# spotify/basic-pitch

Hardware: AMD Instinct MI355X
Metric: audio windows/sec (2 s @ 22.05 kHz) end-to-end CQT+CNN (higher is better)
Workload: dtype f32 I/O + accumulate, split-f16 (22-bit hi+lo) MFMA operands, all three products of every layer on f16 MFMA; 1 GPU; batch=256 synthetic uniform[-1,1) 2 s @ 22.05 kHz mono windows per GPU, fp32, HBM-resident in/out (BASELINE.json configs[1])

## Files before the change

### basic_pitch_amd/_native.py

```python
from __future__ import annotations

import ctypes as C
import os
from typing import Optional

from . import build as _build

BP_OK = 0
BP_ERR_INVALID_ARG = -1
BP_ERR_OUT_OF_MEMORY = -5
BP_ERR_UNSUPPORTED = -6
BP_ERR_BAD_AUDIO = -7
BP_MEM_HOST = 0
BP_MEM_DEVICE = 1
BP_FLAG_STAGE_TIMING = 1
BP_FLAG_TIME_DOMINANT = 16
BP_FLAG_F32_MFMA = 2
BP_FLAG_BF16_WEIGHTS = 4
BP_FLAG_EXT_CQT_44K = 8
BP_FLAG_F16_CORRECTIONS = 32
BP_FLAG_FP8_CORRECTIONS = 64
BP_FLAG_BLOCKING_WAIT = 128
BP_PCM_F32, BP_PCM_S16, BP_PCM_S24, BP_PCM_S32, BP_PCM_U8, BP_PCM_F64 = range(6)
BP_PCM_S16_BE, BP_PCM_S24_BE, BP_PCM_S32_BE, BP_PCM_F32_BE, BP_PCM_F64_BE, BP_PCM_S8, BP_PCM_ULAW, BP_PCM_ALAW = range(6, 14)
# ... 36 lines not shown
        ("compute_units", C.c_int),
        ("max_windows", C.c_int64),
        ("workspace_bytes", C.c_int64),
        ("arch", C.c_char * 32),
    ]


class bp_stage_buffers(C.Structure):
    _fields_ = [
        ("audio", C.c_void_p),
        ("pyr", C.c_void_p),
        ("lp", C.c_void_p),
        ("mm", C.c_void_p),
        ("c1", C.c_void_p),
        ("contour", C.c_void_p),
        ("n1", C.c_void_p),
        ("note", C.c_void_p),
        ("o1", C.c_void_p),
        ("onset", C.c_void_p),
        ("zp", C.c_void_p),
    ]


class bp_launch_plan_out(C.Structure):

    _fields_ = [(name, C.c_int32) for name in (
        "pyramid_one_launch", "pyramid_decimate_grid", "pyramid_decimate_grid_cap", "filterbank_fused", "filterbank_grid",
        "conv1_chunks", "conv1_grid", "conv1_prio", "rim_march", "rim_items", "rim_per_side", "rim_items_max", "rim_items_min",
        "rim_ring", "conv2_slots", "conv2_launches", "conv2_windows", "conv2_first_windows", "conv2_first_groups",
        "conv2_first_slabs", "conv2_first_slab_rows", "conv2_first_grid", "conv2_last_windows", "conv2_last_groups",
        "conv2_last_slabs", "conv2_last_slab_rows", "conv2_last_grid", "note_grid", "note_grid_cap", "note_prio", "note_aligned",
        "note_share_spans_pairs", "onset_grid", "onset_grid_cap", "onset_prio", "onset_aligned", "onset_share_spans_pairs",
        "conv2_fused", "fused_cols", "fused_seam_rows", "fused_term_rows", "fused_window_floats", "finish_slabs",
        "finish_slab_rows", "finish_grid")]


class bp_note_params(C.Structure):
    _fields_ = [
        ("onset_threshold", C.c_double),
        ("frame_threshold", C.c_double),
        ("min_freq_hz", C.c_double),
        ("max_freq_hz", C.c_double),
        ("min_note_len", C.c_int32),
        ("infer_onsets", C.c_int32),
        ("melodia_trick", C.c_int32),
        ("include_pitch_bends", C.c_int32),
        ("energy_tol", C.c_int32),
        ("reserved", C.c_int32),
    ]


class bp_flac_stream_layout(C.Structure):
    _fields_ = [
        ("channels", C.c_int32),
        ("sample_rate", C.c_int32),
        ("bits_per_sample", C.c_int32),
        ("min_block", C.c_int32),
        ("max_block", C.c_int32),
        ("n_frames", C.c_int64),
        ("audio_start", C.c_int64),
    ]


class bp_pcm_file_layout(C.Structure):
    _fields_ = [
        ("container", C.c_int32),
        ("format", C.c_int32),
# ... 659 lines not shown
```

### basic_pitch_amd/csrc/bp_api.hip

```cpp
#include <cmath>
#include <cstring>
#include <ctime>

#include "bp_context.h"
#include "cqt_planes.h"
#include "launch_plan.h"
#include "weight_pack.h"

namespace bp {
static void launch_onset(const uint32_t* zp, const float* note, const void* wfrag, const float* wf32, const void* w16,
                         float* onset, int n_windows, int n_cu, bool weights_have_lo, hipStream_t stream) {
#ifdef BP_AB_KERNELS
  static const int kind = [] {
    const char* e = ab_env("BP_ONSET");
    return e && std::strcmp(e, "ring") == 0 ? 2 : (e && std::strcmp(e, "march32") == 0 ? 1 : 0);
  }();
  if (kind == 1) {
    launch_onset_march(zp, note, wfrag, wf32, onset, n_windows, n_cu, weights_have_lo, stream);
    return;
  }
  if (kind == 2) {
    launch_onset_branch(zp, note, wfrag, wf32, onset, n_windows, n_cu, weights_have_lo, stream);
    return;
  }
// ... 83 lines not shown
static void launch_rim(bp_handle h, const uint32_t* zp, float* c1, int n, bool wlo, hipStream_t s) {
  static const bool gemm = [] {
    const char* e = ab_env("BP_RIM");
    return e && std::strcmp(e, "gemm") == 0;
  }();
  if (h->ext || gemm || !h->d_d1_wrimm)
    launch_contour_conv1_rim(zp, h->d_d1_wrim, h->d_d1_bias.as<float>(), c1, n, h->n_cu, wlo, h->ext, s);
  else
    launch_contour_conv1_rim_march(zp, h->d_d1_wrimm, h->d_d1_bias.as<float>(), c1, n, h->n_cu, wlo, s);
}

static bool contour_fused(bp_handle h) {
  static const bool unfused = [] {
    const char* e = ab_env("BP_CONV2");
    return e && (std::strcmp(e, "unfused") == 0 || std::strcmp(e, "valu") == 0);
  }();
  return !h->ext && !unfused && contour_conv1_use_march();
}

static void launch_conv1_interior(bp_handle h, const uint32_t* zp, float* c1, int n, bool wlo, hipStream_t s) {
#ifdef BP_AB_KERNELS
  if (!contour_conv1_use_march()) {
    launch_contour_conv1_folded(zp, h->d_d1_wfold, h->d_d1_bias.as<float>(), c1, n, h->n_cu, wlo, s);
    return;
  }
#endif
  if (contour_fused(h))
    launch_contour_conv1_march(zp, h->d_d1_wmarch, h->d_d1_bias.as<float>(), h->c1, h->d_d2_w.as<float>(), n, h->n_cu, wlo, s);
  else
    launch_contour_conv1_march(zp, h->d_d1_wmarch, h->d_d1_bias.as<float>(), c1, nullptr, n, h->n_cu, wlo, s);
}

static void launch_conv2_of(bp_handle h, float* contour, int n, bool wlo, hipStream_t s) {
  if (contour_fused(h))
    launch_contour_conv2_finish(h->c1s, h->c1, h->d_d2_wproj, h->b_contour2, contour, n, h->n_cu, wlo, s);
  else
    launch_conv2(h->c1s, h->d_d2_w.as<float>(), h->d_d2_wproj, h->b_contour2, contour, n, h->n_cu, wlo, s);
}

static int64_t pyr_level_off(bp_handle h, int k) {
  return h->ext ? ((k == 1) ? 0 : kAudioN + pyr_off(k - 1)) : pyr_off(k);
}

}

namespace bp {

int run_chunk(bp_handle h, const float* audio_dev, int n, float* note_dev, float* onset_dev,
              float* contour_dev) {
  hipStream_t s = h->stream;
  const bool timing = (h->flags & BP_FLAG_STAGE_TIMING) != 0;
  const bool dom = !timing && (h->flags & BP_FLAG_TIME_DOMINANT) && !(h->flags & BP_FLAG_F32_MFMA) &&
                   (h->dom_chunks++ % bp_context::kDomEvery) == 0;
  const bool wlo = !(h->flags & BP_FLAG_BF16_WEIGHTS);
  int e = dom ? -1 : 0;
  const int ring_slot = (int)(h->timed_chunks % bp_context::kTimedRing);
  hipEvent_t* ev = h->ev[ring_slot];
  int* seq = h->seq[ring_slot];
  if (timing) BP_HIP(hipEventRecord(ev[0], s));
#define BP_DOM_BEGIN()                                \
  do {                                                \
    if (dom) {                                        \
      if (e >= 0) seq[e] = -1;                        \
      BP_HIP(hipEventRecord(ev[e + 1], s));           \
      ++e;                                            \
    }                                                 \
// ... 426 lines not shown
  const PlGeo g = make_pl_geo(ext);
  std::memset(out, 0, sizeof *out);
  out->pyramid_one_launch = pyramid_one_launch(n, n_cu, ext);
  out->pyramid_decimate_grid = out->pyramid_one_launch ? 0 : pyramid_decimate_grid((g.len[1] + kPlTileOut - 1) / kPlTileOut, n, n_cu);
  out->pyramid_decimate_grid_cap = pl_resident_waves(n_cu) / kPlDecimateWaves;
  out->filterbank_fused = filterbank_fused(true, n, n_cu);
  out->filterbank_grid = filterbank_grid(out->filterbank_fused != 0, n, n * g.n_levels * kPlTilesPerLevel, n_cu);
  out->conv1_chunks = contour_march_chunks(n, n_cu);
  out->conv1_grid = contour_march_grid(n * out->conv1_chunks * kCmStrips, n_cu);
  out->conv1_prio = march_prio(kCmPrio, out->conv1_grid, n_cu);
  out->rim_march = !ext;
  if (!ext) {
    out->rim_items = n * kRmTiles;
    out->rim_per_side = rim_march_per_side(out->rim_items, n_cu);
    out->rim_items_max = rim_march_items_of(0, out->rim_items, out->rim_per_side);
    out->rim_items_min = rim_march_items_of(out->rim_per_side - 1, out->rim_items, out->rim_per_side);
    out->rim_ring = kRmRing;
  }
  out->conv2_slots = (int32_t)conv2_proj_slots(n_cu);
  for (int w0 = 0; w0 < n; w0 += kP2PerLaunch) {
    const Conv2ProjLaunch l = conv2_proj_launch(n, w0, n_cu);
    int32_t* dst = w0 == 0 ? &out->conv2_first_windows : &out->conv2_last_windows;
    dst[0] = l.n, dst[1] = l.n_groups, dst[2] = l.n_slabs, dst[3] = l.slab_rows, dst[4] = l.grid;
    if (w0 == 0) std::memcpy(&out->conv2_last_windows, dst, 5 * sizeof(int32_t));
    out->conv2_launches += 1;
    out->conv2_windows += l.n;
  }
  out->conv2_fused = !ext;
  if (!ext) {
    const Conv2FinishLaunch l = conv2_finish_launch(n, n_cu);
    out->fused_cols = kCfCols, out->fused_seam_rows = kCfPrefRows, out->fused_term_rows = kCfTermRows;
    out->fused_window_floats = kCfWin;
    out->finish_slabs = l.n_slabs, out->finish_slab_rows = l.slab_rows, out->finish_grid = l.grid;
  }
  out->note_grid = march_grid(n * kN16Strips, kN16MinFrames, kN16Waves, kN16Occ, n_cu);
  out->note_grid_cap = kN16Occ * n_cu;
  out->note_prio = march_prio(kN16Prio, out->note_grid, n_cu);
  out->note_aligned = march_aligned(out->note_grid * kN16Waves, n * kN16Strips, kN16Strips);
  out->note_share_spans_pairs = march_share_spans_pairs(out->note_grid * kN16Waves, n * kN16Strips, kN16Strips);
  out->onset_grid = march_grid(n * kO16Strips, kO16MinFrames, kO16Waves, kO16Occ, n_cu);
  out->onset_grid_cap = kO16Occ * n_cu;
  out->onset_prio = march_prio(kO16Prio, out->onset_grid, n_cu);
  out->onset_aligned = march_aligned(out->onset_grid * kO16Waves, n * kO16Strips, kO16Strips);
  out->onset_share_spans_pairs = march_share_spans_pairs(out->onset_grid * kO16Waves, n * kO16Strips, kO16Strips);
  return BP_OK;
}

#ifdef BP_AB_KERNELS
int64_t bp_ab_live_device_bytes(void) { return g_live_device_bytes.load(); }
#endif

}
```

### basic_pitch_amd/csrc/bp_kernels.h

```cpp
#pragma once
#include <vector>

#include "bp_common.h"
#include "device_buffer.h"

namespace bp {

void launch_pyramid(const float* audio, float* pyr, const float* lowpass, int n_windows, hipStream_t s);
void launch_window_tracks(const WindowSegs& ts, int n_slots, float* audio, int win_len, int hop, hipStream_t stream);
void launch_unwrap_tracks(const WindowSegs& ts, int n_slots, const float* note, const float* onset, const float* contour,
                          hipStream_t stream);
void launch_window_streams(const WindowSeg* segs, int n_segs, int n_slots, float* audio, int win_len, int hop,
                           hipStream_t stream);
void launch_unwrap_streams(const WindowSeg* segs, int n_segs, int n_slots, const float* note, const float* onset,
                           const float* contour, hipStream_t stream);

size_t filterbank_scratch_floats(int n_windows);
void launch_filterbank(const float* audio, const float* pyr, const float* bfrag, const float* sqrt_len,
                       float* lp, int* mm, float* scratch, int n_windows, LogConsts kc, int n_cu,
                       hipStream_t s);
void launch_mm_reduce(const float* scratch, int* mm, int n_windows, int n_partials, hipStream_t stream);

int64_t planes_elements_per_window(bool ext);
void launch_planes_split(const float* src, int64_t src_stride, int level, uint16_t* pl, int n_windows, bool ext,
// ... 19 lines not shown
void launch_contour2(const float* c1, const float* wgt, float bias, float* contour, int n_windows,
                     hipStream_t s);
void launch_note2(const float* n1, const float* wgt, float bias, float* note, int n_windows,
                  hipStream_t s);
void launch_onset2(const float* note, const float* o1, const float* wgt, float bias, float* onset,
                   int n_windows, hipStream_t s);

void launch_zpack(const float* lp, const int* mm, uint32_t* zp, int n_windows, LogConsts kc, int n_bins,
                  hipStream_t s);
void launch_zpack_partials(const float* lp, const float* scratch, int n_partials, uint32_t* zp, int n_windows,
                           LogConsts kc, int n_bins, hipStream_t stream);

bool contour_conv1_use_march();
void launch_contour_conv1_march(const uint32_t* zp, const void* wfrag, const float* bias, float* c1, const float* w2,
                                int n_windows, int n_cu, bool weights_have_lo, hipStream_t stream);
void launch_contour_conv1_rim(const uint32_t* zp, const void* afrag, const float* bias, float* c1, int n_windows, int n_cu,
                              bool weights_have_lo, bool ext, hipStream_t stream);
void launch_contour_conv1_rim_march(const uint32_t* zp, const void* afrag, const float* bias, float* c1, int n_windows, int n_cu,
                                    bool weights_have_lo, hipStream_t stream);
void launch_contour_conv2_proj(const float* c1, const void* wfrag, float bias, float* contour, int n_windows, int n_cu,
                               bool weights_have_lo, hipStream_t stream);
void launch_contour_conv2_finish(const float* c1s, float* part, const void* wfrag, float bias, float* contour,
                                 int n_windows, int n_cu, bool weights_have_lo, hipStream_t stream);
void launch_note_march16(const float* contour, const void* wfrag, const float* wf32, float* note, int n_windows, int n_cu,
                         bool weights_have_lo, hipStream_t stream);
void launch_onset_march16(const uint32_t* zp, const float* note, const void* wfrag, const float* wf32, float* onset,
                          int n_windows, int n_cu, bool weights_have_lo, hipStream_t stream);

#ifdef BP_AB_KERNELS
void launch_contour_conv1_folded(const uint32_t* zp, const void* wfold, const float* bias, float* c1, int n_windows,
                                 int n_cu, bool weights_have_lo, hipStream_t stream);
void launch_contour_conv2(const float* c1, const float* w2, float bias, float* contour, int n_windows, int n_cu,
                          hipStream_t stream);
void launch_note_march(const float* contour, const void* wfrag, const float* wf32, float* note, int n_windows,
                       bool weights_have_lo, hipStream_t stream);
void launch_onset_march(const uint32_t* zp, const float* note, const void* wfrag, const float* wf32, float* onset,
                        int n_windows, int n_cu, bool weights_have_lo, hipStream_t stream);
void launch_onset_branch(const uint32_t* zp, const float* note, const void* wfrag, const float* wf32, float* onset,
                         int n_windows, int n_cu, bool weights_have_lo, hipStream_t stream);
#endif

ResamplePlan make_resample_plan(int source_rate, int target_rate, std::vector<double>& taps);
void launch_downmix_raw(const void* raw, int format, int64_t n_frames, int channels, float* mono, hipStream_t stream);
void launch_resample(const float* x, int64_t n_in, const double* taps, const ResamplePlan& pl, float* y,
                     int64_t n_out, int mode, hipStream_t stream);
void launch_stream_downmix(const void* raw, int format, int64_t n_frames, int channels, float* dst, int dst_pos, int dst_cap,
                           const float* hist_old, float* hist_new, int n_hist, hipStream_t stream);
void launch_stream_resample(const float* hist, int n_hist, const float* chunk, int64_t chunk_start, int64_t n_in,
                            const double* taps, const ResamplePlan& pl, int64_t k0, int64_t n_k, float* ring, int ring_pos,
                            int ring_cap, hipStream_t stream);

struct ClipDesc {
  const void* src;
  const float* mono;
  float* out;
  int64_t n_frames;
  int64_t n_out;
  int64_t mono_block;
  int64_t out_block;
  int format, channels;
};
void launch_clips_downmix(const ClipDesc* clips, int64_t n_clips, int64_t n_blocks, hipStream_t stream);
void launch_clips_resample(const ClipDesc* clips, int64_t n_clips, int64_t n_blocks, const double* taps, const ResamplePlan& pl,
                           hipStream_t stream);

struct FdStream {
// ... 264 lines not shown
```

### basic_pitch_amd/csrc/conv_contour2.hip

```cpp
#include <stdlib.h>

#include "bp_kernels.h"
#include "launch_plan.h"

namespace bp {


static_assert(kC1Pad == 2, "the pad columns of c1 are the zero padding of the 5-tap rows");

struct Conv2ProjParams {
  const float* c1;
  const uint4* wfrag;
  float bias;
  float* out;
  int n_windows;
  int slab_rows;
  int n_slabs;
};

template <int V>
struct P2Phase {
  static constexpr int v = V;
};

// ... 145 lines not shown
#pragma unroll 1
  for (;;) {
    step(P2Phase<0>{}, rho);
    if (++rho > r_last) break;
    step(P2Phase<1>{}, rho);
    if (++rho > r_last) break;
    step(P2Phase<2>{}, rho);
    if (++rho > r_last) break;
  }
}

void launch_contour_conv2_proj(const float* c1, const void* wfrag, float bias, float* contour, int n_windows, int n_cu,
                               bool weights_have_lo, hipStream_t stream) {
  for (int w0 = 0; w0 < n_windows; w0 += kP2PerLaunch) {
    const Conv2ProjLaunch l = conv2_proj_launch(n_windows, w0, n_cu);
    Conv2ProjParams p{c1 + (int64_t)w0 * kC1Win, static_cast<const uint4*>(wfrag), bias, contour + (int64_t)w0 * kPlaneC, l.n,
                      l.slab_rows, l.n_slabs};
    if (weights_have_lo)
      hipLaunchKernelGGL(contour_conv2_proj_kernel<true>, dim3((unsigned)l.grid), dim3(256), 0, stream, p);
    else
      hipLaunchKernelGGL(contour_conv2_proj_kernel<false>, dim3((unsigned)l.grid), dim3(256), 0, stream, p);
  }
}

struct Conv2FinishParams {
  const float* c1s;
  const float* part;
  const uint4* wfrag;
  float bias;
  float* out;
  int n_windows;
  int slab_rows;
  int n_slabs;
};

template <int R>
__device__ __forceinline__ float cf_seam_class(const float* rec, int cls, int el, bool on) {
  const float* q = rec + 32 * cls + (on ? el : 0);
  float tv[R + 2];
  tv[0] = q[R * kCfClassRow];
#pragma unroll
  for (int i = 0; i <= R; ++i) tv[1 + i] = q[(kCfPrefRows + cf_term_index(R, 4 - R + i)) * kCfClassRow];
  float v = tv[0];
#pragma unroll
  for (int i = 0; i <= R; ++i) v += tv[1 + i];
  return on ? v : 0.0f;
}
template <int R>
__device__ __forceinline__ float cf_seam_col(const float* rec, int col) {
  const bool own = col < 32;
  const float left = cf_seam_class<R>(rec, 2, own ? col - 2 : col - 4, own ? col >= 2 : col >= 34);
  const float mid = cf_seam_class<R>(rec, 1, col, own);
  const float right = cf_seam_class<R>(rec, 0, own ? col + 2 : col - 32, own ? col < 30 : col < 34);
  return (left + mid) + right;
}

__global__ __launch_bounds__(256) void contour_conv2_seam_kernel(float* part, int n_windows, int chunks) {
  const int i = (int)blockIdx.x;
  const int r = i % kCfPrefRows, ci = 1 + (i / kCfPrefRows) % (chunks - 1), b = i / (kCfPrefRows * (chunks - 1));
  const int strip = threadIdx.x / kCfCols, col = threadIdx.x - strip * kCfCols;
  if (b >= n_windows || strip >= kCmStrips) return;
  float* pw = part + (int64_t)b * kCfWin;
  const float* rec = pw + cf_seam_offset(ci, strip);
  const int t = cf_chunk_t0(ci, chunks) - 2 + r;
  float v;
  switch (r) {
    case 0: v = cf_seam_col<0>(rec, col); break;
    case 1: v = cf_seam_col<1>(rec, col); break;
    case 2: v = cf_seam_col<2>(rec, col); break;
    default: v = cf_seam_col<3>(rec, col); break;
  }
  pw[(strip * kFrames + t) * kCfCols + col] = v;
}

template <bool WLO>
__global__ __launch_bounds__(256, kCfOcc) void contour_conv2_finish_kernel(Conv2FinishParams p) {
  const int lane = threadIdx.x & 63;
  const int n = lane & 31, h = lane >> 5;
  const int lblock = (gridDim.x % 8 == 0) ? ((int)blockIdx.x % 8) * ((int)gridDim.x / 8) + (int)blockIdx.x / 8 : (int)blockIdx.x;
  const int64_t wg = (int64_t)lblock * 4 + wave_id();
  if (wg >= (int64_t)p.n_windows * p.n_slabs) return;
  const int b = (int)(wg / p.n_slabs), slab = (int)(wg - (int64_t)b * p.n_slabs);
  const int ta = slab * p.slab_rows;
  const int tb = ta + p.slab_rows < kFrames ? ta + p.slab_rows : kFrames;

  const f16x8 a1 = __builtin_bit_cast(f16x8, p.wfrag[lane]);
  const f16x8 a2 = __builtin_bit_cast(f16x8, WLO ? p.wfrag[64 + lane] : uint4{0u, 0u, 0u, 0u});
  const float* c1w = p.c1s + (int64_t)b * kC1Win;
  const float* partw = p.part + (int64_t)b * kCfWin;
  float* outw = p.out + (int64_t)b * kPlaneC;

  const int src_off[2] = {n * 8 + 4 * h, (236 + n) * 8 + 4 * h};
  const bool ld_ok[2] = {n >= 2 && n <= 21, n >= 10 && n <= 29};
  const int obin[2] = {n - 2, 234 + n};
  const bool st_ok[2] = {h == 1 && n >= 2 && n <= 25, h == 1 && n >= 6 && n <= 29};
  const int rcol[2] = {obin[0] >= 20 ? obin[0] - 20 : (obin[0] >= 18 ? obin[0] + 14 : -1),
                       obin[1] <= 243 ? obin[1] - 212 : (obin[1] <= 245 ? obin[1] - 210 : -1)};
  const bool r_ok[2] = {st_ok[0] && rcol[0] >= 0, st_ok[1] && rcol[1] >= 0};
  const bool i_ok = lane < 54;
  const int ibin = 24 + 4 * (i_ok ? lane : 0);
  const int istrip = (ibin - 20) >> 5, icol = (ibin - 20) & 31;
  const int hal = !i_ok ? 0 : (icol == 0 ? 1 : (icol == 28 ? 2 : 0));
  const int hstrip = hal == 1 ? istrip - 1 : istrip + 1;
  const float* imain = partw + (int64_t)istrip * kFrames * kCfCols + icol;
  const float* ihalo = partw + (int64_t)(hal ? hstrip : istrip) * kFrames * kCfCols + 32;

  const int xhalf4 = (lane ^ 32) * 4;
  int sh4[4];
#pragma unroll
// ... 82 lines not shown
      }
    }
    PartRow q = pbuf[ph];
    pbuf[ph] = loadp(rho + 1);
    if (emit) {
      float y[2] = {V[0][2], V[1][2]};
#pragma unroll
      for (int k = 0; k < 4; ++k) {
        const int df = k < 2 ? k : k + 1;
        y[0] += __builtin_bit_cast(float, __builtin_amdgcn_ds_bpermute(sh4[k], __builtin_bit_cast(int, V[0][df])));
        y[1] += __builtin_bit_cast(float, __builtin_amdgcn_ds_bpermute(sh4[k], __builtin_bit_cast(int, V[1][df])));
      }
      if (hal == 1) q.m.x += q.hq.z, q.m.y += q.hq.w;
      if (hal == 2) q.m.z += q.hq.x, q.m.w += q.hq.y;
      float* orow = outw + (int64_t)t * kFreqC;
      auto sig = [&](float v) { return __builtin_amdgcn_rcpf(1.0f + __builtin_amdgcn_exp2f((v + bias_s) * sig_k)); };
      if (i_ok) *reinterpret_cast<float4*>(orow + ibin) = float4{sig(q.m.x), sig(q.m.y), sig(q.m.z), sig(q.m.w)};
      if (st_ok[0]) orow[obin[0]] = sig(q.r0 + y[0]);
      if (st_ok[1]) orow[obin[1]] = sig(q.r1 + y[1]);
    }
  };
  int rho = r_first;
#pragma unroll 1
  for (;;) {
    step(P2Phase<0>{}, rho);
    if (++rho > r_last) break;
    step(P2Phase<1>{}, rho);
    if (++rho > r_last) break;
    step(P2Phase<2>{}, rho);
    if (++rho > r_last) break;
  }
}

void launch_contour_conv2_finish(const float* c1s, float* part, const void* wfrag, float bias, float* contour,
                                 int n_windows, int n_cu, bool weights_have_lo, hipStream_t stream) {
  if (n_windows <= 0) return;
  const int chunks = contour_march_chunks(n_windows, n_cu);
  hipLaunchKernelGGL(contour_conv2_seam_kernel, dim3((unsigned)(n_windows * (chunks - 1) * kCfPrefRows)), dim3(256), 0, stream,
                     part, n_windows, chunks);
  const Conv2FinishLaunch l = conv2_finish_launch(n_windows, n_cu);
  Conv2FinishParams p{c1s, part, static_cast<const uint4*>(wfrag), bias, contour, n_windows, l.slab_rows, l.n_slabs};
  if (weights_have_lo)
    hipLaunchKernelGGL(contour_conv2_finish_kernel<true>, dim3((unsigned)l.grid), dim3(256), 0, stream, p);
  else
    hipLaunchKernelGGL(contour_conv2_finish_kernel<false>, dim3((unsigned)l.grid), dim3(256), 0, stream, p);
}

#ifdef BP_AB_KERNELS

constexpr int kD2Group = 16;
constexpr int kD2Waves = kD2Group * kC1Row / 64;
static_assert(kD2Group * kC1Row % 64 == 0, "a group of windows fills whole waves");
static_assert(kC1Pad == 2, "the pad columns of c1 are the zero padding of the 5-tap rows");

struct Conv2Params {
  const float* c1;
  const float* w2;
  float bias;
  float* out;
  int n_windows;
  int slab_rows;
  int n_slabs;
};

using v2f = __attribute__((ext_vector_type(2))) float;

__global__ __launch_bounds__(256) void contour_conv2_kernel(const float* __restrict__ c1_, const float* __restrict__ w2_,
                                                            float bias_, float* __restrict__ out_, int n_windows_,
                                                            int slab_rows_, int n_slabs_) {
  const Conv2Params p{c1_, w2_, bias_, out_, n_windows_, slab_rows_, n_slabs_};
  __shared__ __attribute__((aligned(16))) float4 xch[4][2][68];
  const int lane = threadIdx.x & 63;
  const int wv = wave_id();
  const int64_t wg = (int64_t)blockIdx.x * 4 + wv;
  const int n_groups = (p.n_windows + kD2Group - 1) / kD2Group;
  if (wg >= (int64_t)n_groups * p.n_slabs * kD2Waves) return;
  const int seg = (int)(wg % kD2Waves);
  const int slab = (int)((wg / kD2Waves) % p.n_slabs);
  const int group = (int)(wg / ((int64_t)kD2Waves * p.n_slabs));
  const int ta = slab * p.slab_rows;
  const int tb = ta + p.slab_rows < kFrames ? ta + p.slab_rows : kFrames;
// ... 110 lines not shown
```

### basic_pitch_amd/csrc/launch_plan.h

```cpp
#pragma once
#include "march_common.h"

namespace bp {

constexpr int kPlDecimateWaves = 4;
inline int pl_resident_waves(int n_cu) { return n_cu * 16; }
inline bool pyramid_one_launch(int n_windows, int n_cu, bool ext) {
  return ext ? n_windows >= n_cu / 2 : 3 * n_windows >= n_cu;
}
inline int pyramid_decimate_grid(int tiles, int n_windows, int n_cu) {
  const int items = tiles * n_windows;
  int grid = (items + kPlDecimateWaves - 1) / kPlDecimateWaves;
  if (grid > pl_resident_waves(n_cu) / kPlDecimateWaves) grid = pl_resident_waves(n_cu) / kPlDecimateWaves;
  return grid;
}

constexpr int kPlFbThreads = 1024;
inline bool filterbank_fused(bool has_zp, int n_windows, int n_cu) { return has_zp && 2 * n_windows >= n_cu; }
inline int filterbank_grid(bool fused, int n_windows, int tasks, int n_cu) {
  int grid;
  if (fused) {
    grid = n_windows < n_cu ? n_windows : n_cu;
  } else {
    grid = (tasks + kPlFbThreads / 64 - 1) / (kPlFbThreads / 64);
// ... 23 lines not shown

constexpr int kCfCols = 36;
constexpr int kCfClassRow = 3 * 32;
constexpr int kCfPrefRows = 4;
constexpr int kCfTermRows = 10;
constexpr int kCfSeam = (kCfPrefRows + kCfTermRows) * kCfClassRow;
constexpr int kCfMain = kCmStrips * kFrames * kCfCols;
constexpr int kCfWin = kCfMain + (kCmMaxChunks - 1) * kCmStrips * kCfSeam;
static_assert(kCfWin <= 8 * kPlaneC, "the partial sums of a window fit the exact-f32 path's c1 plane, which the default path leaves idle");
__host__ __device__ constexpr int cf_chunk_t0(int ci, int chunks) { return (ci * kFrames) / chunks; }
__host__ __device__ constexpr int cf_chunk_of(int x, int chunks) { return ((x + 1) * chunks - 1) / kFrames; }
__host__ __device__ inline bool cf_seam_of_row(int t, int chunks, int& ci, int& r) {
  const int x = t + 2 < kFrames - 1 ? t + 2 : kFrames - 1;
  ci = cf_chunk_of(x, chunks);
  const int T0 = cf_chunk_t0(ci, chunks);
  r = t - (T0 - 2);
  return ci >= 1 && T0 >= t - 1;
}
__host__ __device__ constexpr int cf_term_index(int r, int dt) { return r * (r + 1) / 2 + dt - (4 - r); }
__host__ __device__ constexpr int64_t cf_seam_offset(int ci, int strip) {
  return (int64_t)kCfMain + (int64_t)((ci - 1) * kCmStrips + strip) * kCfSeam;
}
__host__ __device__ inline bool cf_slot(int gq, int slot, int& dt, int& ob) {
  const int e = gq & 1, s = gq >> 1;
  if (slot < 5) {
    dt = slot, ob = s ? e + 2 : e - 2;
    return true;
  }
  dt = s ? slot - 2 : slot - 5, ob = e;
  return !(s && slot == 7);
}
constexpr int kCfOcc = 2;
constexpr int kCfMaxSlabs = 16;
struct Conv2FinishLaunch {
  int n_slabs, slab_rows, grid;
};
inline Conv2FinishLaunch conv2_finish_launch(int n_windows, int n_cu) {
  Conv2FinishLaunch l;
  int n_slabs = (int)(((int64_t)n_cu * 4 * kCfOcc) / n_windows);
  n_slabs = n_slabs < 1 ? 1 : (n_slabs > kCfMaxSlabs ? kCfMaxSlabs : n_slabs);
  l.slab_rows = (kFrames + n_slabs - 1) / n_slabs;
  l.n_slabs = (kFrames + l.slab_rows - 1) / l.slab_rows;
  l.grid = (int)(((int64_t)n_windows * l.n_slabs + 3) / 4);
  return l;
}

constexpr int kRmTileFrames = 16;
constexpr int kRmTiles = (kFrames + kRmTileFrames - 1) / kRmTileFrames;
#ifndef BP_RM_DEPTH
#define BP_RM_DEPTH 4
#endif
constexpr int kRmDepth = BP_RM_DEPTH;
constexpr int kRmRing = kRmDepth + 1;
inline int rim_march_per_side(int n_items, int n_cu) {
  int per_side = n_cu / 2 > 0 ? n_cu / 2 : 1;
  if (per_side > n_items) per_side = n_items;
  return per_side;
}
inline int rim_march_items_of(int wg, int n_items, int per_side) {
  return wg < n_items ? (n_items - wg + per_side - 1) / per_side : 0;
}

constexpr int kP2Group = 16;
constexpr int kP2Cols = kP2Group * kC1Row;
constexpr int kP2Strip = 64, kP2Stride = 60;
constexpr int kP2Strips = (kP2Cols + kP2Stride - 1) / kP2Stride;
#ifndef P2_OCC
#define P2_OCC 4
#endif
constexpr int kP2Occ = P2_OCC;
constexpr int kP2PerLaunch = 256;
constexpr int kP2MaxSlabs = 16;
struct Conv2ProjLaunch {
  int n;
  int n_groups;
  int n_slabs;
// ... 40 lines not shown
```

### include/basic_pitch_amd.h

```cpp
#ifndef BASIC_PITCH_AMD_H
#define BASIC_PITCH_AMD_H

#include <stddef.h>
#include <stdint.h>

#ifdef __cplusplus
extern "C" {
#endif

#define BP_AUDIO_SAMPLE_RATE 22050
#define BP_FFT_HOP 256
#define BP_AUDIO_N_SAMPLES 43844
#define BP_N_FRAMES 172
#define BP_N_BINS_CQT 309
#define BP_N_FREQ_CONTOUR 264
#define BP_N_FREQ_NOTE 88
#define BP_N_OVERLAP_FRAMES 30
#define BP_OVERLAP_LEN 7680
#define BP_HOP_SIZE 36164
#define BP_FRAMES_PER_WINDOW 142

typedef struct bp_context* bp_handle;

typedef enum bp_status {
// ... 174 lines not shown
  int32_t rim_items_min;
  int32_t rim_ring;
  int32_t conv2_slots;
  int32_t conv2_launches;
  int32_t conv2_windows;
  int32_t conv2_first_windows;
  int32_t conv2_first_groups;
  int32_t conv2_first_slabs;
  int32_t conv2_first_slab_rows;
  int32_t conv2_first_grid;
  int32_t conv2_last_windows;
  int32_t conv2_last_groups;
  int32_t conv2_last_slabs;
  int32_t conv2_last_slab_rows;
  int32_t conv2_last_grid;
  int32_t note_grid;
  int32_t note_grid_cap;
  int32_t note_prio;
  int32_t note_aligned;
  int32_t note_share_spans_pairs;
  int32_t onset_grid;
  int32_t onset_grid_cap;
  int32_t onset_prio;
  int32_t onset_aligned;
  int32_t onset_share_spans_pairs;
  int32_t conv2_fused;
  int32_t fused_cols;
  int32_t fused_seam_rows;
  int32_t fused_term_rows;
  int32_t fused_window_floats;
  int32_t finish_slabs;
  int32_t finish_slab_rows;
  int32_t finish_grid;
} bp_launch_plan_out;
int bp_launch_plan(int64_t n_windows, int n_cu, unsigned flags, bp_launch_plan_out* out);

int bp_pyramid_layout(int level , int64_t* offset, int64_t* length);

const char* bp_version(void);
int bp_device_count(void);

typedef struct bp_note_params {
  double onset_threshold;
  double frame_threshold;
  double min_freq_hz;
  double max_freq_hz;
  int32_t min_note_len;
  int32_t infer_onsets;
  int32_t melodia_trick;
  int32_t include_pitch_bends;
  int32_t energy_tol;
  int32_t reserved;
} bp_note_params;

typedef struct bp_note_event {
  double start_s, end_s;
  int64_t bend_offset;
  int32_t start_frame, end_frame;
  int32_t pitch_midi;
  int32_t n_bends;
  float amplitude;
  int32_t reserved;
} bp_note_event;

void bp_note_params_default(bp_note_params* p);

// ... 64 lines not shown
```

Measured before the change: 395,300 windows/s.

## Split contour conv2 finish into rim-MFMA and streaming sigmoid roles

Restructures the fused contour conv2 finish kernel into two roles in one launch. Rim blocks recompute only the edge frequency bins with MFMA and a register-ring prefetch. Stream blocks read the precomputed partial sums with batched float4 loads, add halo corrections and apply the sigmoid. The aim is to stop every block from carrying the full MFMA register and latency cost when most output bins only need a memory-bound finish, which raises occupancy for the streaming part. The cost is a heterogeneous grid, more plan fields and extra complexity in the halo indexing. The old kernel is kept as an A/B option.

```diff
diff --git a/basic_pitch_amd/_native.py b/basic_pitch_amd/_native.py
--- a/basic_pitch_amd/_native.py
+++ b/basic_pitch_amd/_native.py
@@ -92,7 +92,7 @@
         "conv2_last_slabs", "conv2_last_slab_rows", "conv2_last_grid", "note_grid", "note_grid_cap", "note_prio", "note_aligned",
         "note_share_spans_pairs", "onset_grid", "onset_grid_cap", "onset_prio", "onset_aligned", "onset_share_spans_pairs",
         "conv2_fused", "fused_cols", "fused_seam_rows", "fused_term_rows", "fused_window_floats", "finish_slabs",
-        "finish_slab_rows", "finish_grid")]
+        "finish_slab_rows", "finish_grid", "finish_stream_runs", "finish_stream_rows", "finish_stream_grid")]
 
 
 class bp_note_params(C.Structure):
diff --git a/basic_pitch_amd/csrc/bp_api.hip b/basic_pitch_amd/csrc/bp_api.hip
--- a/basic_pitch_amd/csrc/bp_api.hip
+++ b/basic_pitch_amd/csrc/bp_api.hip
@@ -139,6 +139,16 @@
 }
 
 static void launch_conv2_of(bp_handle h, float* contour, int n, bool wlo, hipStream_t s) {
+#ifdef BP_AB_KERNELS
+  static const bool finish1 = [] {
+    const char* e = ab_env("BP_CONV2");
+    return e && std::strcmp(e, "finish1") == 0;
+  }();
+  if (finish1 && contour_fused(h)) {
+    launch_contour_conv2_finish1(h->c1s, h->c1, h->d_d2_wproj, h->b_contour2, contour, n, h->n_cu, wlo, s);
+    return;
+  }
+#endif
   if (contour_fused(h))
     launch_contour_conv2_finish(h->c1s, h->c1, h->d_d2_wproj, h->b_contour2, contour, n, h->n_cu, wlo, s);
   else
@@ -631,6 +641,8 @@
     out->fused_cols = kCfCols, out->fused_seam_rows = kCfPrefRows, out->fused_term_rows = kCfTermRows;
     out->fused_window_floats = kCfWin;
     out->finish_slabs = l.n_slabs, out->finish_slab_rows = l.slab_rows, out->finish_grid = l.grid;
+    const Conv2StreamLaunch ls = conv2_stream_launch(n, n_cu);
+    out->finish_stream_runs = ls.n_runs, out->finish_stream_rows = ls.run_rows, out->finish_stream_grid = ls.grid;
   }
   out->note_grid = march_grid(n * kN16Strips, kN16MinFrames, kN16Waves, kN16Occ, n_cu);
   out->note_grid_cap = kN16Occ * n_cu;
diff --git a/basic_pitch_amd/csrc/bp_kernels.h b/basic_pitch_amd/csrc/bp_kernels.h
--- a/basic_pitch_amd/csrc/bp_kernels.h
+++ b/basic_pitch_amd/csrc/bp_kernels.h
@@ -75,6 +75,8 @@
                                  int n_cu, bool weights_have_lo, hipStream_t stream);
 void launch_contour_conv2(const float* c1, const float* w2, float bias, float* contour, int n_windows, int n_cu,
                           hipStream_t stream);
+void launch_contour_conv2_finish1(const float* c1s, float* part, const void* wfrag, float bias, float* contour,
+                                  int n_windows, int n_cu, bool weights_have_lo, hipStream_t stream);
 void launch_note_march(const float* contour, const void* wfrag, const float* wf32, float* note, int n_windows,
                        bool weights_have_lo, hipStream_t stream);
 void launch_onset_march(const uint32_t* zp, const float* note, const void* wfrag, const float* wf32, float* onset,
diff --git a/basic_pitch_amd/csrc/conv_contour2.hip b/basic_pitch_amd/csrc/conv_contour2.hip
--- a/basic_pitch_amd/csrc/conv_contour2.hip
+++ b/basic_pitch_amd/csrc/conv_contour2.hip
@@ -201,6 +201,10 @@
   int n_windows;
   int slab_rows;
   int n_slabs;
+  int rim_grid;
+  int n_runs;
+  int run_rows;
+  int stream_grid;
 };
 
 template <int R>
@@ -242,8 +246,280 @@
   pw[(strip * kFrames + t) * kCfCols + col] = v;
 }
 
+constexpr int kCfRimRole = 1, kCfStreamRole = 2;
+
+__device__ __forceinline__ int cf_role_block(int lb, int grid) { return (grid % 8 == 0) ? (lb % 8) * (grid / 8) + lb / 8 : lb; }
+
 template <bool WLO>
-__global__ __launch_bounds__(256, kCfOcc) void contour_conv2_finish_kernel(Conv2FinishParams p) {
+__device__ __forceinline__ void cf_rim_role(const Conv2FinishParams& p, int lb) {
+  const int lane = threadIdx.x & 63;
+  const int n = lane & 31, h = lane >> 5;
+  const int64_t wg = (int64_t)cf_role_block(lb, p.rim_grid) * 4 + wave_id();
+  if (wg >= (int64_t)p.n_windows * p.n_slabs) return;
+  const int b = (int)(wg / p.n_slabs), slab = (int)(wg - (int64_t)b * p.n_slabs);
+  const int ta = slab * p.slab_rows;
+  const int tb = ta + p.slab_rows < kFrames ? ta + p.slab_rows : kFrames;
+
+  const f16x8 a1 = __builtin_bit_cast(f16x8, p.wfrag[lane]);
+  const f16x8 a2 = __builtin_bit_cast(f16x8, WLO ? p.wfrag[64 + lane] : uint4{0u, 0u, 0u, 0u});
+  const float* c1w = p.c1s + (int64_t)b * kC1Win;
+  const float* partw = p.part + (int64_t)b * kCfWin;
+  float* outw = p.out + (int64_t)b * kPlaneC;
+
+  const int nc[2] = {n < 2 ? 2 : (n > 21 ? 21 : n), n < 10 ? 10 : (n > 29 ? 29 : n)};
+  const int src_off[2] = {nc[0] * 8 + 4 * h, (236 + nc[1]) * 8 + 4 * h};
+  const bool ld_ok[2] = {n >= 2 && n <= 21, n >= 10 && n <= 29};
+  const int obin[2] = {n - 2, 234 + n};
+  const bool st_ok[2] = {h == 1 && n >= 2 && n <= 25, h == 1 && n >= 6 && n <= 29};
+  const int rcol[2] = {obin[0] >= 20 ? obin[0] - 20 : (obin[0] >= 18 ? obin[0] + 14 : -1),
+                       obin[1] <= 243 ? obin[1] - 212 : (obin[1] <= 245 ? obin[1] - 210 : -1)};
+  const bool r_ok[2] = {st_ok[0] && rcol[0] >= 0, st_ok[1] && rcol[1] >= 0};
+
+  const int xhalf4 = (lane ^ 32) * 4;
+  int sh4[4];
+#pragma unroll
+  for (int k = 0; k < 4; ++k) sh4[k] = (32 + ((n + (k < 2 ? k - 2 : k - 1)) & 31)) * 4;
+  const float bias_s = p.bias * kLoScale;
+  const float sig_k = -1.44269504088896341f * kLoUnscale;
+  const float hmask = h ? 1.0f : 0.0f;
+
+  float X0[2][5], X1[2][5], IN[2][5];
+#pragma unroll
+  for (int tl = 0; tl < 2; ++tl)
+#pragma unroll
+    for (int df = 0; df < 5; ++df) X0[tl][df] = X1[tl][df] = IN[tl][df] = 0.0f;
+
+  constexpr int kRowFloats = kC1Row * 8;
+  auto load = [&](int rho, int tl) {
+    const int rc = rho < 0 ? 0 : (rho > kFrames - 1 ? kFrames - 1 : rho);
+    return *reinterpret_cast<const float4*>(c1w + (int64_t)rc * kRowFloats + src_off[tl]);
+  };
+  auto pixel = [&](float4 v, int tl) {
+    return ld_ok[tl] ? v : float4{0.0f, 0.0f, 0.0f, 0.0f};
+  };
+  struct PartRow {
+    float r0, r1;
+  };
+  const int pcol[2] = {r_ok[0] ? rcol[0] : 0, r_ok[1] ? rcol[1] : 0};
+  auto loadp = [&](int t) {
+    const int tc = t < 0 ? 0 : (t > kFrames - 1 ? kFrames - 1 : t);
+    PartRow q;
+    q.r0 = partw[tc * kCfCols + pcol[0]];
+    q.r1 = partw[((kCmStrips - 1) * kFrames + tc) * kCfCols + pcol[1]];
+    return q;
+  };
+  const int r_first = ta - 2, r_last = tb + 1;
+  float4 buf[kCfDepth][2];
+  PartRow pbuf[kCfDepth];
+#pragma unroll
+  for (int k = 0; k < kCfDepth; ++k) {
+#pragma unroll
+    for (int tl = 0; tl < 2; ++tl) buf[k][tl] = load(r_first + k, tl);
+    pbuf[k] = loadp(r_first + k - 2);
+  }
+
+  auto step = [&](auto PH, int rho) {
+    constexpr int ph = decltype(PH)::v;
+    const int t = rho - 2;
+    const bool emit = t >= ta && t < tb;
+    float V[2][5];
+    if (rho >= 0 && rho < kFrames) {
+      f16x8 bq[2];
+#pragma unroll
+      for (int tl = 0; tl < 2; ++tl) {
+        uint32_t h01, l01, h23, l23;
+        const float4 px = pixel(buf[ph][tl], tl);
+        split_f16x2(f32x2{px.x, px.y}, h01, l01);
+        split_f16x2(f32x2{px.z, px.w}, h23, l23);
+        bq[tl] = __builtin_bit_cast(f16x8, uint4{h01, h23, l01, l23});
+        buf[ph][tl] = load(rho + kCfDepth, tl);
+      }
+#pragma unroll
+      for (int tl = 0; tl < 2; ++tl) {
+        const f32x16 zero16 = {0.f, 0.f, 0.f, 0.f, 0.f, 0.f, 0.f, 0.f, 0.f, 0.f, 0.f, 0.f, 0.f, 0.f, 0.f, 0.f};
+        f32x16 P = __builtin_amdgcn_mfma_f32_32x32x16_f16(a1, bq[tl], zero16, 0, 0, 0);
+        if (WLO) P = __builtin_amdgcn_mfma_f32_32x32x16_f16(a2, bq[tl], P, 0, 0, 0);
+#pragma unroll
+        for (int df = 0; df < 5; ++df) {
+          const float x2 = X1[tl][df] + P[10 + df];
+          const float x1 = X0[tl][df] + P[5 + df];
+          X0[tl][df] = __builtin_fmaf(IN[tl][df], hmask, P[df]);
+          X1[tl][df] = x1;
+          V[tl][df] = x1;
+          IN[tl][df] = __builtin_bit_cast(float, __builtin_amdgcn_ds_bpermute(xhalf4, __builtin_bit_cast(int, x2)));
+        }
+      }
+    } else {
+#pragma unroll
+      for (int tl = 0; tl < 2; ++tl) {
+        buf[ph][tl] = load(rho + kCfDepth, tl);
+#pragma unroll
+        for (int df = 0; df < 5; ++df) {
+          const float x2 = X1[tl][df];
+          V[tl][df] = X1[tl][df] = X0[tl][df];
+          X0[tl][df] = IN[tl][df] * hmask;
+          IN[tl][df] = __builtin_bit_cast(float, __builtin_amdgcn_ds_bpermute(xhalf4, __builtin_bit_cast(int, x2)));
+        }
+      }
+    }
+    const PartRow q = pbuf[ph];
+    pbuf[ph] = loadp(rho + kCfDepth - 2);
+    if (emit) {
+      float y[2] = {V[0][2], V[1][2]};
+#pragma unroll
+      for (int k = 0; k < 4; ++k) {
+        const int df = k < 2 ? k : k + 1;
+        y[0] += __builtin_bit_cast(float, __builtin_amdgcn_ds_bpermute(sh4[k], __builtin_bit_cast(int, V[0][df])));
+        y[1] += __builtin_bit_cast(float, __builtin_amdgcn_ds_bpermute(sh4[k], __builtin_bit_cast(int, V[1][df])));
+      }
+      float* orow = outw + (int64_t)t * kFreqC;
+      auto sig = [&](float v) { return __builtin_amdgcn_rcpf(1.0f + __builtin_amdgcn_exp2f((v + bias_s) * sig_k)); };
+      if (st_ok[0]) orow[obin[0]] = sig((r_ok[0] ? q.r0 : 0.0f) + y[0]);
+      if (st_ok[1]) orow[obin[1]] = sig((r_ok[1] ? q.r1 : 0.0f) + y[1]);
+    }
+  };
+  static_assert(kCfDepth >= 3 && kCfDepth <= 6, "the loop below is written out for three to six register sets");
+  int rho = r_first;
+#pragma unroll 1
+  for (;;) {
+    step(P2Phase<0>{}, rho);
+    if (++rho > r_last) break;
+    step(P2Phase<1>{}, rho);
+    if (++rho > r_last) break;
+    step(P2Phase<2>{}, rho);
+    if (++rho > r_last) break;
+    if constexpr (kCfDepth > 3) {
+      step(P2Phase<3>{}, rho);
+      if (++rho > r_last) break;
+    }
+    if constexpr (kCfDepth > 4) {
+      step(P2Phase<4>{}, rho);
+      if (++rho > r_last) break;
+    }
+    if constexpr (kCfDepth > 5) {
+      step(P2Phase<5>{}, rho);
+      if (++rho > r_last) break;
+    }
+  }
+}
+
+__device__ __forceinline__ void cf_stream_role(const Conv2FinishParams& p, int lb) {
+  const int lane = threadIdx.x & 63;
+  const int64_t wg = (int64_t)cf_role_block(lb, p.stream_grid) * 4 + wave_id();
+  if (wg >= (int64_t)p.n_windows * p.n_runs) return;
+  const int b = (int)(wg / p.n_runs), run = (int)(wg - (int64_t)b * p.n_runs);
+  const int ta = run * p.run_rows;
+  const int tb = ta + p.run_rows < kFrames ? ta + p.run_rows : kFrames;
+  const int total = (tb - ta) * kCfGroups;
+  const float* partw = p.part + (int64_t)b * kCfWin;
+  float* outw = p.out + (int64_t)b * kPlaneC;
+  const float bias_s = p.bias * kLoScale;
+  const float sig_k = -1.44269504088896341f * kLoUnscale;
+
+  struct El {
+    float4 m;
+    f32x2 hq;
+  };
+  El set[2][kCfStreamU];
+  const int row_l = lane >= kCfGroups ? 1 : 0, g_l = lane - row_l * kCfGroups;
+  auto where = [&](int e0, uint32_t& t, uint32_t& bin, uint32_t& strip, uint32_t& icol) {
+    const int q0 = e0 / kCfGroups, r0 = e0 - q0 * kCfGroups;
+    const int g1 = g_l + r0, row1 = q0 + row_l;
+    const bool carry = g1 >= kCfGroups, past = e0 + lane >= total;
+    const int g = past ? kCfGroups - 1 : (carry ? g1 - kCfGroups : g1);
+    const int row = past ? tb - ta - 1 : (carry ? row1 + 1 : row1);
+    t = (uint32_t)(ta + row), bin = 24 + 4 * (uint32_t)g;
+    strip = (bin - 20) >> 5, icol = (bin - 20) & 31;
+  };
+  const char* partb = reinterpret_cast<const char*>(partw);
+  char* outb = reinterpret_cast<char*>(outw);
+  auto issue = [&](El (&s)[kCfStreamU], int e0) {
+#pragma unroll
+    for (int u = 0; u < kCfStreamU; ++u) {
+      uint32_t t, bin, strip, icol;
+      where(e0 + 64 * u, t, bin, strip, icol);
+      s[u].m = *reinterpret_cast<const float4*>(partb + ((strip * kFrames + t) * kCfCols + icol) * 4u);
+      const uint32_t hstrip = icol == 0 ? strip - 1 : (icol == 28 ? strip + 1 : strip);
+      const uint32_t hcol = icol == 0 ? 34 : (icol == 28 ? 32 : icol);
+      s[u].hq = *reinterpret_cast<const f32x2*>(partb + ((hstrip * kFrames + t) * kCfCols + hcol) * 4u);
+    }
+  };
+  auto finish = [&](El (&s)[kCfStreamU], int e0) {
+#pragma unroll
+    for (int u = 0; u < kCfStreamU; ++u) {
+      uint32_t t, bin, strip, icol;
+      where(e0 + 64 * u, t, bin, strip, icol);
+      float4 v = s[u].m;
+      const float fx = v.x + s[u].hq.x, fy = v.y + s[u].hq.y, bz = v.z + s[u].hq.x, bw = v.w + s[u].hq.y;
+      v.x = icol == 0 ? fx : v.x, v.y = icol == 0 ? fy : v.y;
+      v.z = icol == 28 ? bz : v.z, v.w = icol == 28 ? bw : v.w;
+      auto sig = [&](float x) { return __builtin_amdgcn_rcpf(1.0f + __builtin_amdgcn_exp2f((x + bias_s) * sig_k)); };
+      if (e0 + 64 * u + lane < total)
+        *reinterpret_cast<float4*>(outb + (t * kFreqC + bin) * 4u) = float4{sig(v.x), sig(v.y), sig(v.z), sig(v.w)};
+    }
+  };
+  constexpr int kBatch = 64 * kCfStreamU;
+  int e0 = 0;
+  issue(set[0], 0);
+#pragma unroll 1
+  do {
+    issue(set[1], e0 + kBatch);
+    __builtin_amdgcn_sched_barrier(0);
+    finish(set[0], e0);
+    issue(set[0], e0 + 2 * kBatch);
+    __builtin_amdgcn_sched_barrier(0);
+    finish(set[1], e0 + kBatch);
+    e0 += 2 * kBatch;
+  } while (e0 < total);
+}
+
+template <bool WLO, int ROLES>
+__global__ __launch_bounds__(256, ROLES == kCfStreamRole ? kCfStreamOcc : kCfRegOcc) void contour_conv2_finish_kernel(Conv2FinishParams p) {
+  const int bid = (int)blockIdx.x;
+  if (ROLES == kCfRimRole) {
+    cf_rim_role<WLO>(p, bid);
+  } else if (ROLES == kCfStreamRole) {
+    cf_stream_role(p, bid);
+  } else if (bid < p.rim_grid) {
+    cf_rim_role<WLO>(p, bid);
+  } else {
+    cf_stream_role(p, bid - p.rim_grid);
+  }
+}
+
+static void launch_contour_conv2_seam(float* part, int n_windows, int n_cu, hipStream_t stream) {
+  const int chunks = contour_march_chunks(n_windows, n_cu);
+  hipLaunchKernelGGL(contour_conv2_seam_kernel, dim3((unsigned)(n_windows * (chunks - 1) * kCfPrefRows)), dim3(256), 0, stream,
+                     part, n_windows, chunks);
+}
+
+void launch_contour_conv2_finish(const float* c1s, float* part, const void* wfrag, float bias, float* contour,
+                                 int n_windows, int n_cu, bool weights_have_lo, hipStream_t stream) {
+  if (n_windows <= 0) return;
+  launch_contour_conv2_seam(part, n_windows, n_cu, stream);
+  const Conv2FinishLaunch l = conv2_finish_launch(n_windows, n_cu);
+  const Conv2StreamLaunch ls = conv2_stream_launch(n_windows, n_cu);
+  Conv2FinishParams p{c1s, part, static_cast<const uint4*>(wfrag), bias, contour, n_windows, l.slab_rows, l.n_slabs,
+                      l.grid, ls.n_runs, ls.run_rows, ls.grid};
+#ifdef CF_TWO_LAUNCHES
+  hipLaunchKernelGGL((contour_conv2_finish_kernel<true, kCfStreamRole>), dim3((unsigned)ls.grid), dim3(256), 0, stream, p);
+  if (weights_have_lo)
+    hipLaunchKernelGGL((contour_conv2_finish_kernel<true, kCfRimRole>), dim3((unsigned)l.grid), dim3(256), 0, stream, p);
+  else
+    hipLaunchKernelGGL((contour_conv2_finish_kernel<false, kCfRimRole>), dim3((unsigned)l.grid), dim3(256), 0, stream, p);
+#else
+  const dim3 grid((unsigned)(l.grid + ls.grid));
+  if (weights_have_lo)
+    hipLaunchKernelGGL((contour_conv2_finish_kernel<true, kCfRimRole | kCfStreamRole>), grid, dim3(256), 0, stream, p);
+  else
+    hipLaunchKernelGGL((contour_conv2_finish_kernel<false, kCfRimRole | kCfStreamRole>), grid, dim3(256), 0, stream, p);
+#endif
+}
+
+#ifdef BP_AB_KERNELS
+
+template <bool WLO>
+__global__ __launch_bounds__(256, kCfOcc) void contour_conv2_finish1_kernel(Conv2FinishParams p) {
   const int lane = threadIdx.x & 63;
   const int n = lane & 31, h = lane >> 5;
   const int lblock = (gridDim.x % 8 == 0) ? ((int)blockIdx.x % 8) * ((int)gridDim.x / 8) + (int)blockIdx.x / 8 : (int)blockIdx.x;
@@ -392,21 +668,18 @@
   }
 }
 
-void launch_contour_conv2_finish(const float* c1s, float* part, const void* wfrag, float bias, float* contour,
-                                 int n_windows, int n_cu, bool weights_have_lo, hipStream_t stream) {
+void launch_contour_conv2_finish1(const float* c1s, float* part, const void* wfrag, float bias, float* contour,
+                                  int n_windows, int n_cu, bool weights_have_lo, hipStream_t stream) {
   if (n_windows <= 0) return;
-  const int chunks = contour_march_chunks(n_windows, n_cu);
-  hipLaunchKernelGGL(contour_conv2_seam_kernel, dim3((unsigned)(n_windows * (chunks - 1) * kCfPrefRows)), dim3(256), 0, stream,
-                     part, n_windows, chunks);
+  launch_contour_conv2_seam(part, n_windows, n_cu, stream);
   const Conv2FinishLaunch l = conv2_finish_launch(n_windows, n_cu);
   Conv2FinishParams p{c1s, part, static_cast<const uint4*>(wfrag), bias, contour, n_windows, l.slab_rows, l.n_slabs};
   if (weights_have_lo)
-    hipLaunchKernelGGL(contour_conv2_finish_kernel<true>, dim3((unsigned)l.grid), dim3(256), 0, stream, p);
+    hipLaunchKernelGGL(contour_conv2_finish1_kernel<true>, dim3((unsigned)l.grid), dim3(256), 0, stream, p);
   else
-    hipLaunchKernelGGL(contour_conv2_finish_kernel<false>, dim3((unsigned)l.grid), dim3(256), 0, stream, p);
-}
-
-#ifdef BP_AB_KERNELS
+    hipLaunchKernelGGL(contour_conv2_finish1_kernel<false>, dim3((unsigned)l.grid), dim3(256), 0, stream, p);
+}
+
 
 constexpr int kD2Group = 16;
 constexpr int kD2Waves = kD2Group * kC1Row / 64;
diff --git a/basic_pitch_amd/csrc/launch_plan.h b/basic_pitch_amd/csrc/launch_plan.h
--- a/basic_pitch_amd/csrc/launch_plan.h
+++ b/basic_pitch_amd/csrc/launch_plan.h
@@ -79,6 +79,24 @@
 }
 constexpr int kCfOcc = 2;
 constexpr int kCfMaxSlabs = 16;
+#ifndef CF_REG_OCC
+#define CF_REG_OCC 4
+#endif
+#ifndef CF_DEPTH
+#define CF_DEPTH 3
+#endif
+#ifndef CF_STREAM_U
+#define CF_STREAM_U 4
+#endif
+#ifndef CF_STREAM_OCC
+#define CF_STREAM_OCC 4
+#endif
+constexpr int kCfRegOcc = CF_REG_OCC;
+constexpr int kCfDepth = CF_DEPTH;
+constexpr int kCfGroups = 54;
+constexpr int kCfStreamU = CF_STREAM_U;
+constexpr int kCfStreamOcc = CF_STREAM_OCC;
+constexpr int kCfMaxRuns = 16;
 struct Conv2FinishLaunch {
   int n_slabs, slab_rows, grid;
 };
@@ -89,6 +107,18 @@
   l.slab_rows = (kFrames + n_slabs - 1) / n_slabs;
   l.n_slabs = (kFrames + l.slab_rows - 1) / l.slab_rows;
   l.grid = (int)(((int64_t)n_windows * l.n_slabs + 3) / 4);
+  return l;
+}
+struct Conv2StreamLaunch {
+  int n_runs, run_rows, grid;
+};
+inline Conv2StreamLaunch conv2_stream_launch(int n_windows, int n_cu) {
+  Conv2StreamLaunch l;
+  int n_runs = (int)(((int64_t)n_cu * 4 * kCfStreamOcc) / n_windows);
+  n_runs = n_runs < 1 ? 1 : (n_runs > kCfMaxRuns ? kCfMaxRuns : n_runs);
+  l.run_rows = (kFrames + n_runs - 1) / n_runs;
+  l.n_runs = (kFrames + l.run_rows - 1) / l.run_rows;
+  l.grid = (int)(((int64_t)n_windows * l.n_runs + 3) / 4);
   return l;
 }
 
diff --git a/include/basic_pitch_amd.h b/include/basic_pitch_amd.h
--- a/include/basic_pitch_amd.h
+++ b/include/basic_pitch_amd.h
@@ -230,6 +230,9 @@
   int32_t finish_slabs;
   int32_t finish_slab_rows;
   int32_t finish_grid;
+  int32_t finish_stream_runs;
+  int32_t finish_stream_rows;
+  int32_t finish_stream_grid;
 } bp_launch_plan_out;
 int bp_launch_plan(int64_t n_windows, int n_cu, unsigned flags, bp_launch_plan_out* out);
 
```

New measurement: 384,700 windows/s. -2.7%, worse.
